# pinterest/rocksplicator

Hardware: AMD Instinct MI355X
Metric: replicated updates/sec (Put+Delete) at 1024 shards (higher is better)
Workload: dtype u8; 1 GPU; 1024shards_16Bkey_1024Bval_zipf0.99; key_len=16, val_len=1024, tick_updates=819200, parallelism=shard-parallel x1

## Files before the change

### rocksplicator_amd/csrc/engine.hip

```cpp
#include <hip/hip_runtime.h>

#define WB_UNALIGNED_OK 1

#include <algorithm>
#include <atomic>
#include <chrono>
#include <cstdio>
#include <cstring>
#include <deque>
#include <map>
#include <memory>
#include <mutex>
#include <string>
#include <thread>
#include <vector>

#include "../../include/rocksplicator_gpu.h"
#include "dev_buf.h"
#include "fold.h"
#include "host_store.h"
#include "part_copy.h"
#include "snappy.h"
#include "wb_format.h"

static thread_local std::string g_err;
extern "C" const char *gra_last_error(void) { return g_err.c_str(); }

#define HIP_TRY(x)                                                     \
  do {                                                                 \
    hipError_t _e = (x);                                               \
    if (_e != hipSuccess) {                                            \
      g_err = std::string(#x) + ": " + hipGetErrorString(_e);          \
      return GRA_ERR;                                                  \
    }                                                                  \
  } while (0)

namespace gra {

struct UpdDesc {
  uint64_t off;
  uint64_t base_seq;
  uint32_t len;
  uint32_t shard;
};
struct TickPlace {
  uint64_t cur;
  uint64_t hdr_off;
  uint64_t payload_off;
  uint64_t payload_bytes;
  uint32_t total_rec;
  uint32_t overflow;
};
struct SnapTask {
  uint64_t comp_off;
  uint64_t out_off;
  uint32_t comp_len;
  uint32_t ulen;
};
struct GroupDesc {
  uint32_t shard, first, n_upds, _pad;
};
struct DevRunDesc {
  uint64_t base_seq, last_seq;
  uint64_t cur;
  uint64_t hdr_off, payload_off;
  uint32_t n_entries, payload_bytes;
  uint32_t pay_rel_base;
  uint32_t shard;
};

__host__ __device__ inline uint2 add2(uint2 a, uint2 b) {
  return make_uint2(a.x + b.x, a.y + b.y);
}


constexpr uint32_t kSnapStage = 508;

__global__ void __launch_bounds__(256) k_snappy(
    const uint8_t *__restrict__ comp, const SnapTask *__restrict__ tasks,
    uint32_t n, uint8_t *__restrict__ scratch,
    uint32_t *__restrict__ err_ring, uint32_t tick) {
  __shared__ uint8_t lds[256 * (kSnapStage + 4)];
  uint32_t i = blockIdx.x * blockDim.x + threadIdx.x;
  if (i >= n) return;
  SnapTask t = tasks[i];
  uint8_t *dst = scratch + t.out_off;
  uint32_t r;
  if (t.comp_len <= kSnapStage) {
    uint8_t *mine = lds + threadIdx.x * (kSnapStage + 4);
    const uint8_t *src = comp + t.comp_off;
    for (uint32_t b = 0; b < t.comp_len; b += 16)
      *(uint4 *)(mine + b) = *(const uint4 *)(src + b);
    r = snp::decompress(mine, t.comp_len, dst, t.ulen);
  } else {
    r = snp::decompress(comp + t.comp_off, t.comp_len, dst, t.ulen);
  }
  if (r != t.ulen) {
    for (int b = 0; b < 13; b++) dst[b] = 0xFF;
    atomicAdd(&err_ring[tick % 64u], 1u);
  }
}

constexpr uint32_t kErrRing = 64;

constexpr uint32_t kRecCache = 2;

__device__ __forceinline__ uint2 block_scan256(uint2 v, uint2 *total) {
  __shared__ uint2 wsum[4];
  const uint32_t lane = threadIdx.x & 63u, w = threadIdx.x >> 6;
  uint2 inc = v;
  for (int ofs = 1; ofs < 64; ofs <<= 1) {
    uint32_t x = __shfl_up(inc.x, ofs, 64), y = __shfl_up(inc.y, ofs, 64);
    if (lane >= (uint32_t)ofs) inc = add2(inc, make_uint2(x, y));
  }
  if (lane == 63) wsum[w] = inc;
  __syncthreads();
  uint2 before = make_uint2(0, 0), tot = make_uint2(0, 0);
  for (uint32_t k = 0; k < 4; k++) {
    uint2 s = wsum[k];
    if (k < w) before = add2(before, s);
    tot = add2(tot, s);
  }
  *total = tot;
  return make_uint2(before.x + inc.x - v.x, before.y + inc.y - v.y);
}

constexpr uint32_t kDecodeWin = 48;
static_assert(kDecodeWin % 16 == 0, "window is staged in 16 B chunks");

__global__ void __launch_bounds__(256) k_decode(
    const uint8_t *__restrict__ blobs, const UpdDesc *__restrict__ descs,
    uint32_t n, wb::WalkTotals *__restrict__ totals, uint32_t max_rec,
    uint32_t *__restrict__ err_ring, uint32_t tick,
    uint2 *__restrict__ partial, uint2 *__restrict__ bsums,
    wb::Rec *__restrict__ reccache, uint8_t *__restrict__ ok_out) {
  __shared__ uint32_t stage[256 * (kDecodeWin + 4) / 4];
  uint32_t i = blockIdx.x * 256 + threadIdx.x;
  uint2 v = make_uint2(0, 0);
  if (i < n) {
    UpdDesc d = descs[i];
    const uint8_t *rep = blobs + d.off;
    uint32_t *row = stage + threadIdx.x * ((kDecodeWin + 4) / 4);
    const uint32_t nch = wb::win_chunks(d.len, kDecodeWin);
    uint4 c[kDecodeWin / 16];
#pragma unroll
    for (uint32_t k = 0; k < kDecodeWin / 16; k++)
      if (k < nch) c[k] = *(const uint4 *)(rep + 16 * k);
#pragma unroll
    for (uint32_t k = 0; k < kDecodeWin / 16; k++)
      if (k < nch) {
        row[4 * k + 0] = c[k].x;
        row[4 * k + 1] = c[k].y;
        row[4 * k + 2] = c[k].z;
        row[4 * k + 3] = c[k].w;
      }
    wb::WinSrc src = {(const uint8_t *)row, wb::win_bytes(d.len, kDecodeWin),
                      rep};
    wb::Rec *cache = reccache + (size_t)i * kRecCache;
    wb::WalkTotals t = wb::walk_src(src, d.len,
                                    [&](const wb::Rec &r, uint32_t idx) {
                                      if (idx < kRecCache) cache[idx] = r;
                                    });
    if (t.n_records > max_rec) t.ok = 0;
    totals[i] = t;
    ok_out[i] = (uint8_t)t.ok;
    if (!t.ok) atomicAdd(&err_ring[tick % kErrRing], 1u);
    if (t.ok) v = make_uint2(t.n_records, t.payload16);
  }
  uint2 tot;
  uint2 excl = block_scan256(v, &tot);
  if (i < n) partial[i] = excl;
  if (threadIdx.x == 255) bsums[blockIdx.x] = tot;
}

__global__ void k_scan2(uint2 *__restrict__ bsums, uint32_t nblocks,
                        uint64_t *__restrict__ cursor,
                        TickPlace *__restrict__ place, uint64_t cap, int ring,
                        uint32_t task_cap, uint32_t *__restrict__ err_ring,
                        uint32_t tick) {
  const uint32_t per = (nblocks + 255) / 256;
  const uint32_t lo = threadIdx.x * per < nblocks ? threadIdx.x * per : nblocks;
  const uint32_t hi = lo + per < nblocks ? lo + per : nblocks;
  uint2 mine = make_uint2(0, 0);
  for (uint32_t i = lo; i < hi; i++) mine = add2(mine, bsums[i]);
  uint2 carry;
  uint2 run = block_scan256(mine, &carry);
  for (uint32_t i = lo; i < hi; i++) {
    uint2 v = bsums[i];
    bsums[i] = run;
    run = add2(run, v);
  }
  if (threadIdx.x == 0) {
    bsums[nblocks] = carry;
    uint2 tot = carry;
    uint64_t need_hdr = (((uint64_t)tot.x * sizeof(wb::RecHdr)) + 15) & ~15ULL;
    uint64_t need_pay = tot.y;
    uint64_t need = need_hdr + need_pay;
    TickPlace p = {};
    p.total_rec = tot.x;
    p.payload_bytes = need_pay;
    uint64_t cur = *cursor;
    if ((cur % cap) + need > cap) cur += cap - (cur % cap);
    if (need > cap || (!ring && cur + need > cap) ||
        (uint64_t)tot.x * 2 > task_cap) {
      p.overflow = 1;
      p.total_rec = 0;
      atomicAdd(&err_ring[tick % kErrRing], 1u);
    } else {
      p.cur = cur;
      p.hdr_off = cur % cap;
      p.payload_off = (cur % cap) + need_hdr;
      *cursor = cur + need;
    }
    *place = p;
    err_ring[(tick + kErrRing / 2) % kErrRing] = 0;
  }
}

__global__ void k_emit(const uint8_t *__restrict__ blobs,
                       const UpdDesc *__restrict__ descs, uint32_t n,
                       const wb::WalkTotals *__restrict__ totals,
                       const uint2 *__restrict__ partial,
                       const uint2 *__restrict__ bsums,
                       const TickPlace *__restrict__ place,
                       uint8_t *__restrict__ store,
                       CopyTask *__restrict__ tasks,
                       const wb::Rec *__restrict__ reccache) {
  uint32_t i = blockIdx.x * blockDim.x + threadIdx.x;
  if (i >= n) return;
  if (place->overflow) return;
  wb::WalkTotals t = totals[i];
  if (!t.ok || t.n_records == 0) return;
  UpdDesc d = descs[i];
  uint2 base = add2(partial[i], bsums[i >> 8]);
  wb::RecHdr *hdrs = (wb::RecHdr *)(store + place->hdr_off);
  uint8_t *pay_region = store + place->payload_off;
  uint32_t pay = base.y;
  uint32_t rec = base.x;
  auto emit_one = [&](const wb::Rec &r, uint32_t idx) {
    uint32_t cf4 = r.cf_id ? 4u : 0u;
    uint8_t btag = wb::base_tag(r.tag);
    uint32_t cfv = (cf4 && btag == wb::kRangeDeletion) ? 4u : 0u;
    wb::RecHdr h;
    h.seq = d.base_seq + idx;
    h.kv_off = pay;
    h.val_len = r.val_len + cfv;
    h.key_len = (uint16_t)(r.key_len + cf4);
    h.type = btag;
    h.flags = cf4 ? 1 : 0;
    h.kpref = 0;
    hdrs[rec + idx] = h;
    if (cf4) {
      *(uint32_t *)(pay_region + pay) = r.cf_id;
    }
    CopyTask tk;
    tk.src_off = d.off + r.key_off;
    tk.dst_rel = pay + cf4;
    tk.nbytes = r.key_len;
    tasks[2 * (rec + idx)] = tk;
    if (cfv) {
      uint8_t *p = pay_region + pay + cf4 + r.key_len;
      p[0] = (uint8_t)r.cf_id;
      p[1] = (uint8_t)(r.cf_id >> 8);
      p[2] = (uint8_t)(r.cf_id >> 16);
      p[3] = (uint8_t)(r.cf_id >> 24);
    }
    tk.src_off = d.off + r.val_off;
    tk.dst_rel = pay + cf4 + r.key_len + cfv;
    tk.nbytes = r.val_len;
    tasks[2 * (rec + idx) + 1] = tk;
    pay += (cf4 + r.key_len + cfv + r.val_len + 15u) & ~15u;
  };
  if (t.n_records <= kRecCache) {
    const wb::Rec *cache = reccache + (size_t)i * kRecCache;
    for (uint32_t idx = 0; idx < t.n_records; idx++) emit_one(cache[idx], idx);
  } else {
    wb::walk_f(blobs + d.off, d.len, emit_one);
  }
}

template <int G>
__device__ __forceinline__ void copy_dword(uint8_t *dst, const uint8_t *src,
                                           uint32_t n, uint32_t lane) {
  uint32_t head = (uint32_t)((0u - (uint32_t)(uintptr_t)dst) & 3u);
  if (head > n) head = n;
  if (lane < head) dst[lane] = src[lane];
  dst += head;
  src += head;
  n -= head;
  uint32_t nw = n >> 2;
  uint32_t r = (uint32_t)((uintptr_t)src & 3);
  const uint32_t *asrc = (const uint32_t *)(src - r);
  uint32_t *adst = (uint32_t *)dst;
  if (r == 0) {
    for (uint32_t w = lane; w < nw; w += G) adst[w] = asrc[w];
  } else {
    uint32_t sh = 8 * r;
    for (uint32_t w = lane; w < nw; w += G)
      adst[w] = (asrc[w] >> sh) | (asrc[w + 1] << (32 - sh));
  }
  uint32_t done = nw << 2, tail = n & 3;
  if (lane < tail) dst[done + lane] = src[done + lane];
}

template <int G, int R, bool UNAL>
__global__ void __launch_bounds__(256) k_copy(const uint8_t *__restrict__ blobs,
                                              uint8_t *__restrict__ store,
                                              const TickPlace *__restrict__ place,
                                              const CopyTask *__restrict__ tasks) {
  if (place->overflow) return;
  uint32_t wave = (blockIdx.x * blockDim.x + threadIdx.x) >> 6;
  uint32_t nwaves = (gridDim.x * blockDim.x) >> 6;
  pcopy::part_copy<G, R, UNAL>(blobs, store + place->payload_off, tasks,
                               place->total_rec, wave, nwaves);
}

__global__ void k_drain(const uint8_t *__restrict__ store,
                        const TickPlace *__restrict__ place,
                        uint8_t *__restrict__ hostbuf) {
  if (place->overflow) return;
  uint64_t hdr_bytes = (uint64_t)place->total_rec * sizeof(wb::RecHdr);
  uint64_t hb16 = (hdr_bytes + 15) & ~15ull;
  uint64_t pay = place->payload_bytes;
  const uint8_t *hsrc = store + place->hdr_off;
  const uint8_t *psrc = store + place->payload_off;
  size_t stride = (size_t)gridDim.x * blockDim.x * 16;
  size_t i0 = ((size_t)blockIdx.x * blockDim.x + threadIdx.x) * 16;
  for (size_t b = i0; b < hdr_bytes; b += stride)
    *(uint4 *)(hostbuf + b) = *(const uint4 *)(hsrc + b);
  uint8_t *pdst = hostbuf + hb16;
  for (size_t b = i0; b < pay; b += stride)
    *(uint4 *)(pdst + b) = *(const uint4 *)(psrc + b);
}

__global__ void k_rundesc(const GroupDesc *__restrict__ groups, uint32_t ngroups,
                          const UpdDesc *__restrict__ descs,
                          const wb::WalkTotals *__restrict__ totals,
                          const uint2 *__restrict__ partial,
                          const uint2 *__restrict__ bsums, uint32_t n,
                          uint32_t nblocks,
                          const TickPlace *__restrict__ place,
                          DevRunDesc *__restrict__ out) {
  uint32_t g = blockIdx.x * blockDim.x + threadIdx.x;
  if (g >= ngroups) return;
  GroupDesc gd = groups[g];
  auto scan_at = [&](uint32_t j) {
    return j >= n ? bsums[nblocks] : add2(partial[j], bsums[j >> 8]);
  };
  uint2 s0 = scan_at(gd.first);
  uint2 s1 = scan_at(gd.first + gd.n_upds);
  DevRunDesc rd = {};
  rd.shard = gd.shard;
  rd.n_entries = s1.x - s0.x;
  rd.payload_bytes = s1.y - s0.y;
  rd.pay_rel_base = s0.y;
  if (!place->overflow) {
    rd.cur = place->cur;
    rd.hdr_off = place->hdr_off + (uint64_t)s0.x * sizeof(wb::RecHdr);
    rd.payload_off = place->payload_off + s0.y;
    rd.base_seq = descs[gd.first].base_seq;
    const UpdDesc last = descs[gd.first + gd.n_upds - 1];
    rd.last_seq = last.base_seq + totals[gd.first + gd.n_upds - 1].hdr_count - 1;
  } else {
    rd.n_entries = 0;
  }
  out[g] = rd;
}

#include "mg_kernels.h"

#include "scan_kernels.h"

#include "compact_kernels.h"

#include "reclaim_kernels.h"

__host__ __device__ inline uint64_t rec_hash_cs(uint64_t seq, uint8_t type,
                                                uint32_t klen, uint32_t vlen,
                                                const uint8_t *key,
                                                const uint8_t *val) {
  uint64_t h = 1469598103934665603ULL;
#define GRA_FOLD(b) h = (h ^ (uint8_t)(b)) * 1099511628211ULL
  for (int i = 0; i < 8; i++) GRA_FOLD(seq >> (8 * i));
  GRA_FOLD(type);
  for (int i = 0; i < 4; i++) GRA_FOLD(klen >> (8 * i));
  for (int i = 0; i < 4; i++) GRA_FOLD(vlen >> (8 * i));
  for (uint32_t i = 0; i < klen; i++) GRA_FOLD(key[i]);
  for (uint32_t i = 0; i < vlen; i++) GRA_FOLD(val[i]);
#undef GRA_FOLD
  return h;
}

__global__ void k_checksum(const uint8_t *__restrict__ store,
                           const RunView *__restrict__ runs, uint32_t nruns,
                           unsigned long long *__restrict__ out) {
  uint64_t local = 0;
  for (uint32_t r = blockIdx.x; r < nruns; r += gridDim.x) {
    RunView rv = runs[r];
    const wb::RecHdr *hdrs = (const wb::RecHdr *)(store + rv.hdr_off);
    const uint8_t *pay = store + rv.payload_off;
    for (uint32_t i = threadIdx.x; i < rv.n_entries; i += blockDim.x) {
      wb::RecHdr h = hdrs[i];
      uint32_t rel = h.kv_off - rv.pay_rel_base;
      local += rec_hash_cs(h.seq, h.type, h.key_len, h.val_len, pay + rel,
                           pay + rel + h.key_len);
    }
  }
  for (int ofs = 32; ofs > 0; ofs >>= 1)
    local += __shfl_down(local, ofs, 64);
  if ((threadIdx.x & 63) == 0 && local)
    atomicAdd(out, (unsigned long long)local);
}

static bool env_flag(const char *name) {
  const char *v = getenv(name);
  return v && v[0] == '1';
}

static bool gra_check_staging() {
  static const bool on = env_flag("GRA_CHECK_STAGING");
  return on;
}


struct Stats {
  double h2d_ms = 0, snappy_ms = 0, decode_ms = 0, scan_ms = 0, emit_ms = 0,
         copy_ms = 0, runfix_ms = 0, total_ms = 0;
  uint64_t ticks = 0, updates = 0, records = 0, blob_bytes = 0, payload_bytes = 0;
};

constexpr int kSlots = 8;
enum TickEvent {
  kEvTickStart,
  kEvH2dStart,
  kEvH2dDone,
  kEvSnappyStart,
  kEvSnappyDone,
  kEvAfterDecode,
  kEvAfterScan,
  kEvAfterEmit,
  kEvAfterCopy,
  kEvMainEnd,
  kEvPublished,
  kEventsPerTick
};

struct TickRec {
  int slot = -1;
  uint32_t n = 0, ngroups = 0;
  uint64_t blob_bytes = 0;
  uint32_t evmask = 0;
  std::vector<uint32_t> counts;
  std::shared_ptr<uint8_t> drain_buf;
  hipEvent_t ev[kEventsPerTick];

  hipError_t record(TickEvent k, hipStream_t s) {
    evmask |= bit(k);
    return hipEventRecord(ev[k], s);
  }
  bool has(TickEvent k) const { return evmask & bit(k); }
  static uint32_t bit(TickEvent k) { return 1u << k; }
};

struct TickInput {
  uint32_t n = 0;
  const std::vector<GroupDesc> *groups = nullptr;
  const GroupDesc *d_groups = nullptr;
  uint64_t blob_bytes = 0;
  std::vector<uint32_t> counts;
  const uint8_t *d_blobs = nullptr;
  const UpdDesc *d_descs = nullptr;
  const void *stage_src = nullptr;
  size_t stage_bytes = 0;
  const UpdDesc *h_descs = nullptr;
  const uint8_t *d_comp = nullptr;
  const SnapTask *d_snaptasks = nullptr;
  hipEvent_t window_ev = nullptr;
};

struct Slot {
  GroupDesc *h_groups = nullptr;
  TickPlace *h_place = nullptr;
  DevRunDesc *h_rundescs = nullptr;
  DevRunDesc *d_rundescs = nullptr;
  uint8_t *d_ok = nullptr;
  uint8_t *h_ok = nullptr;
  uint32_t *h_err = nullptr;
  UpdDesc *h_descs = nullptr;
  bool busy = false;
};

}

using namespace gra;

struct GraEngine {
  GraEngineOpts opts;
  hipStream_t stream = nullptr;
  hipStream_t copyout = nullptr;
  hipStream_t h2d = nullptr;
  hipStream_t prep = nullptr;
  uint8_t *d_store = nullptr;
  uint64_t *d_cursor = nullptr;
  uint32_t max_upd;
  uint32_t task_cap;
  uint32_t copy_grid;
  uint32_t group_cap;
  wb::WalkTotals *d_totals = nullptr;
  uint2 *d_partial = nullptr;
  uint2 *d_bsums = nullptr;
  wb::Rec *d_reccache = nullptr;
  CopyTask *d_tasks = nullptr;
  TickPlace *d_place = nullptr;
  GroupDesc *d_groups = nullptr;
  uint32_t *d_err_ring = nullptr;
  uint32_t tick_id = 0;
  static constexpr int kWriterSlots = 256;
  struct WriterSlot {
    alignas(64) std::atomic<uint32_t> n{0};
  };
  struct StageBuf {
    uint8_t *pin = nullptr;
    GraUpdateDesc *descs = nullptr;
    alignas(64) std::atomic<uint64_t> pos{0};
    alignas(64) std::atomic<uint32_t> nslots{0};
    alignas(64) std::atomic<bool> closed{false};
    alignas(64) std::atomic<uint32_t> staged{0};
    WriterSlot writers[kWriterSlots];
    uint64_t epoch = 0;
    hipEvent_t free_ev = nullptr;
  };
  StageBuf stage[2];
  std::atomic<StageBuf *> cur_stage{nullptr};
  uint8_t *d_stage_blobs_bufs[2] = {nullptr, nullptr};
  UpdDesc *d_stage_descs_bufs[2] = {nullptr, nullptr};
  hipEvent_t stage_used_ev[2] = {nullptr, nullptr};
  hipEvent_t h2d_gate_ev[2] = {nullptr, nullptr};
  Slot slots[kSlots];
  std::deque<TickRec> pending;
  std::vector<hipEvent_t> event_pool;
  struct MgCounts {
    uint32_t ncand, ntomb;
  };
  struct MgCache {
    DevBuf<RunView> d_runs;
    DevBuf<GraKeyRef> d_keys;
    DevBuf<uint8_t> d_keybuf, d_valbuf;
    DevBuf<GraGetResult> d_out;
    DevBuf<MgExtra> d_extra;
    DevBuf<uint64_t> d_qtab;
    DevBuf<MgCand> d_cands;
    DevBuf<MgTomb> d_tombs;
    DevBuf<unsigned long long> d_aux;
    DevMirror<MgCounts> counts;
  } mg;
  struct ScCache {
    DevBuf<RunView> d_runs;
    DevBuf<uint8_t> d_bounds, d_out;
    DevBuf<ScCand> d_cands;
    DevBuf<ScTomb> d_tombs;
    DevBuf<ScItem> d_items;
    DevBuf<ScHead> d_heads;
    DevBuf<ScFold> d_folds;
    DevBuf<ScSum> d_bsums;
    DevBuf<GraScanEntry> d_ents;
    DevMirror<ScCtl> ctl;
    DevMirror<CpCtl> cp;
    uint32_t cand_cap = 0;
  } sc;
  std::mutex drain_mu;
  std::vector<std::pair<uint8_t *, size_t>> drain_pool;
  bool closing = false;
  std::shared_ptr<uint8_t> drain_alloc(size_t need);
  std::vector<ShardState> shards;
  Stats stats;
  std::mutex mu;
  std::mutex maint_mu;
  std::atomic<uint64_t> store_epoch{0};
  uint64_t rc_bounce_bytes = 0, rc_piece_bytes = 0;
  DevBuf<uint8_t> rc_bounce;
  DevBuf<RcTask> rc_tasks;

  int init(const GraEngineOpts &o);
  ~GraEngine();
  int enqueue_tick(TickInput &in);
  int ingest(bool wait_all);
  int ingest_one(TickRec &t, bool wait);
  int flush_locked();
  int stream_tick_locked();
  hipEvent_t get_event();
  void put_event(hipEvent_t e);
  int free_slot();
};

struct GraDb {
  GraEngine *e;
  uint32_t shard;
};

struct TickPlan {
  std::vector<GroupDesc> groups;
  uint64_t blob_bytes = 0;
  GroupDesc *d_groups = nullptr;
  UpdDesc *d_ud = nullptr;
  hipEvent_t consumed_ev = nullptr;
  SnapTask *d_snap = nullptr;
};

struct GraReplay {
  GraEngine *e = nullptr;
  uint8_t *d_blobs = nullptr;
  bool external_blobs = false;
  UpdDesc *d_descs = nullptr;
  std::vector<UpdDesc> descs;
  std::vector<uint16_t> counts;
  size_t arena_bytes = 0;
  const uint8_t *h_arena = nullptr;
  uint8_t *d_comp = nullptr;
  SnapTask *d_snaptasks = nullptr;
  std::vector<SnapTask> snap_tasks;
  bool snappy = false;
  std::map<std::pair<uint64_t, uint64_t>, TickPlan> plans;
};

std::shared_ptr<uint8_t> GraEngine::drain_alloc(size_t need) {
  uint8_t *p = nullptr;
  size_t cap = 0;
  {
    std::lock_guard<std::mutex> lk(drain_mu);
    for (auto it = drain_pool.begin(); it != drain_pool.end(); ++it) {
      if (it->second >= need) {
        p = it->first;
        cap = it->second;
        drain_pool.erase(it);
        break;
      }
    }
  }
  if (!p) {
    cap = need + 64;
    if (hipHostMalloc(&p, cap) != hipSuccess) return nullptr;
  }
  GraEngine *e = this;
  return std::shared_ptr<uint8_t>(p, [e, cap](uint8_t *q) {
    std::lock_guard<std::mutex> lk(e->drain_mu);
    if (e->closing) {
      (void)hipHostFree(q);
    } else {
      e->drain_pool.push_back({q, cap});
    }
  });
}

hipEvent_t GraEngine::get_event() {
  if (!event_pool.empty()) {
    hipEvent_t e = event_pool.back();
    event_pool.pop_back();
    return e;
  }
  hipEvent_t e;
  (void)hipEventCreate(&e);
  return e;
}
void GraEngine::put_event(hipEvent_t e) { event_pool.push_back(e); }

int GraEngine::init(const GraEngineOpts &o) {
  opts = o;
  if (opts.store_bytes == 0) opts.store_bytes = 4ULL << 30;
  if (opts.staging_bytes == 0) opts.staging_bytes = 256ULL << 20;
  if (opts.max_wb_records == 0) opts.max_wb_records = 1024;
  max_upd = 1u << 20;
  task_cap = 4u << 20;
  copy_grid = 2048;
  if (const char *g = getenv("GRA_COPY_GRID")) {
    long v = atol(g);
    copy_grid = (uint32_t)(v < 1 ? 1 : v > 2048 ? 2048 : v);
  }
  rc_bounce_bytes = 64ull << 20;
  rc_piece_bytes = 16u << 20;
  if (const char *g = getenv("GRA_RECLAIM_BOUNCE"))
    rc_bounce_bytes = strtoull(g, nullptr, 10);
  if (const char *g = getenv("GRA_RECLAIM_PIECE"))
    rc_piece_bytes = strtoull(g, nullptr, 10);
  group_cap = opts.nshards + 1 > 65536 ? opts.nshards + 1 : 65536;
  (void)hipGetLastError();
  int ndev = 0;
  hipError_t de = hipGetDeviceCount(&ndev);
  if (de != hipSuccess || ndev == 0) {
    g_err = "no HIP device present — the GPU apply path refuses to run "
            "(no CPU fallback by design)";
    return GRA_NO_GPU;
  }
  if (opts.device >= 0) {
    hipError_t se = hipSetDevice(opts.device);
    if (se != hipSuccess) {
      g_err = std::string("hipSetDevice: ") + hipGetErrorString(se);
      (void)hipGetLastError();
      return GRA_ERR;
    }
  }
  HIP_TRY(hipStreamCreate(&stream));
  HIP_TRY(hipStreamCreate(&copyout));
  HIP_TRY(hipStreamCreate(&h2d));
  HIP_TRY(hipStreamCreate(&prep));
  HIP_TRY(hipMalloc(&d_store, opts.store_bytes + 16));
  HIP_TRY(hipMalloc(&d_cursor, 8));
  HIP_TRY(hipMemset(d_cursor, 0, 8));
  HIP_TRY(hipMalloc(&d_totals, (size_t)max_upd * sizeof(wb::WalkTotals)));
  HIP_TRY(hipMalloc(&d_partial, (size_t)max_upd * sizeof(uint2)));
  HIP_TRY(hipMalloc(&d_bsums, ((size_t)max_upd / 256 + 2) * sizeof(uint2)));
  HIP_TRY(hipMalloc(&d_reccache, (size_t)max_upd * 2 * sizeof(wb::Rec)));
  HIP_TRY(hipMalloc(&d_tasks, (size_t)task_cap * sizeof(CopyTask)));
  HIP_TRY(hipMalloc(&d_place, kSlots * sizeof(TickPlace)));
  HIP_TRY(hipMalloc(&d_groups, (size_t)group_cap * sizeof(GroupDesc)));
  HIP_TRY(hipMalloc(&d_err_ring, kErrRing * 4));
  HIP_TRY(hipMemset(d_err_ring, 0, kErrRing * 4));
  for (int i = 0; i < 2; i++) {
    HIP_TRY(hipMalloc(&d_stage_blobs_bufs[i], opts.staging_bytes + 16));
    HIP_TRY(hipMalloc(&d_stage_descs_bufs[i], (size_t)max_upd * sizeof(UpdDesc)));
    HIP_TRY(hipEventCreate(&stage_used_ev[i]));
    HIP_TRY(hipEventRecord(stage_used_ev[i], stream));
    HIP_TRY(hipEventCreateWithFlags(&h2d_gate_ev[i], hipEventDisableTiming));
    HIP_TRY(hipEventRecord(h2d_gate_ev[i], h2d));
  }
  static std::atomic<uint64_t> g_epoch{1};
  for (int i = 0; i < 2; i++) {
    HIP_TRY(hipHostMalloc(&stage[i].pin, opts.staging_bytes + 16,
                          hipHostMallocNonCoherent));
    stage[i].descs = (GraUpdateDesc *)malloc((size_t)max_upd * sizeof(GraUpdateDesc));
    stage[i].epoch = g_epoch.fetch_add(1u << 20);
    HIP_TRY(hipEventCreate(&stage[i].free_ev));
    HIP_TRY(hipEventRecord(stage[i].free_ev, stream));
  }
  cur_stage.store(&stage[0]);
  for (int i = 0; i < kSlots; i++) {
    Slot &s = slots[i];
    HIP_TRY(hipHostMalloc(&s.h_groups, (size_t)group_cap * sizeof(GroupDesc)));
    HIP_TRY(hipHostMalloc(&s.h_place, sizeof(TickPlace)));
    HIP_TRY(hipHostMalloc(&s.h_rundescs, (size_t)group_cap * sizeof(DevRunDesc)));
    HIP_TRY(hipMalloc(&s.d_rundescs, (size_t)group_cap * sizeof(DevRunDesc)));
    HIP_TRY(hipMalloc(&s.d_ok, (size_t)max_upd));
    HIP_TRY(hipHostMalloc(&s.h_ok, (size_t)max_upd));
    HIP_TRY(hipHostMalloc(&s.h_err, 4));
    HIP_TRY(hipHostMalloc(&s.h_descs, (size_t)max_upd * sizeof(UpdDesc)));
  }
  if (opts.drain_host && opts.store_ring &&
      opts.store_bytes < 10 * opts.staging_bytes) {
    g_err = "drain_host with store_ring needs store_bytes >= 10x "
            "staging_bytes (ring wrap inside the drain pipeline)";
    return GRA_ERR;
  }
  shards = std::vector<ShardState>(opts.nshards);
  event_pool.reserve(kSlots * kEventsPerTick);
  for (int i = 0; i < kSlots * kEventsPerTick; i++) {
    hipEvent_t ev;
    HIP_TRY(hipEventCreate(&ev));
    event_pool.push_back(ev);
  }
  return GRA_OK;
}

GraEngine::~GraEngine() {
  {
    std::lock_guard<std::mutex> lk(drain_mu);
    closing = true;
  }
  (void)hipStreamSynchronize(stream);
  (void)hipStreamSynchronize(copyout);
  (void)hipStreamSynchronize(h2d);
  for (auto &t : pending)
    for (int i = 0; i < kEventsPerTick; i++)
      if (t.ev[i]) (void)hipEventDestroy(t.ev[i]);
  for (auto e : event_pool) (void)hipEventDestroy(e);
  for (int i = 0; i < 2; i++) {
    if (stage[i].pin) (void)hipHostFree(stage[i].pin);
    free(stage[i].descs);
    if (stage[i].free_ev) (void)hipEventDestroy(stage[i].free_ev);
  }
  for (int i = 0; i < kSlots; i++) {
    Slot &s = slots[i];
    if (s.h_groups) (void)hipHostFree(s.h_groups);
    if (s.h_place) (void)hipHostFree(s.h_place);
    if (s.h_rundescs) (void)hipHostFree(s.h_rundescs);
    if (s.d_rundescs) (void)hipFree(s.d_rundescs);
    if (s.d_ok) (void)hipFree(s.d_ok);
    if (s.h_ok) (void)hipHostFree(s.h_ok);
    if (s.h_err) (void)hipHostFree(s.h_err);
    if (s.h_descs) (void)hipHostFree(s.h_descs);
  }
  for (int i = 0; i < 2; i++) {
    if (d_stage_blobs_bufs[i]) (void)hipFree(d_stage_blobs_bufs[i]);
    if (d_stage_descs_bufs[i]) (void)hipFree(d_stage_descs_bufs[i]);
    if (stage_used_ev[i]) (void)hipEventDestroy(stage_used_ev[i]);
    if (h2d_gate_ev[i]) (void)hipEventDestroy(h2d_gate_ev[i]);
  }
  for (void *p : {(void *)d_totals, (void *)d_partial, (void *)d_bsums,
                  (void *)d_reccache, (void *)d_store, (void *)d_cursor,
                  (void *)d_tasks,
                  (void *)d_place, (void *)d_groups, (void *)d_err_ring})
    if (p) (void)hipFree(p);
  shards.clear();
  pending.clear();
  {
    std::lock_guard<std::mutex> lk(drain_mu);
    for (auto &pr : drain_pool) (void)hipHostFree(pr.first);
    drain_pool.clear();
  }
  if (stream) (void)hipStreamDestroy(stream);
  if (copyout) (void)hipStreamDestroy(copyout);
  if (h2d) (void)hipStreamDestroy(h2d);
  if (prep) (void)hipStreamDestroy(prep);
}

int GraEngine::free_slot() {
  for (;;) {
    for (int i = 0; i < kSlots; i++)
      if (!slots[i].busy) return i;
    int rc = ingest(false);
    if (rc != GRA_OK) return -1;
    if (!pending.empty()) {
      if (ingest_one(pending.front(), true) != GRA_OK) return -1;
      pending.pop_front();
    }
  }
}

int GraEngine::enqueue_tick(TickInput &in) {
  const uint32_t n = in.n;
  const uint64_t blob_bytes = in.blob_bytes;
  const std::vector<GroupDesc> &groups = *in.groups;
  if (n == 0) return GRA_OK;
  if (n > max_upd) {
    g_err = "tick exceeds max updates per tick";
    return GRA_ERR;
  }
  if (opts.drain_host && opts.store_ring && blob_bytes * 10 > opts.store_bytes) {
    g_err = "drain_host with store_ring needs store_bytes >= 10x the tick "
            "size (ring wrap inside the drain pipeline)";
    return GRA_ERR;
  }
  if (groups.size() > group_cap) {
    g_err = "tick exceeds max shard-groups per tick";
    return GRA_ERR;
  }
  int si = free_slot();
  if (si < 0) return GRA_ERR;
  Slot &sl = slots[si];
  sl.busy = true;
  uint32_t ngroups = (uint32_t)groups.size();
  memcpy(sl.h_groups, groups.data(), ngroups * sizeof(GroupDesc));
  const GroupDesc *groups_for_kernel = in.d_groups ? in.d_groups : d_groups;
  uint32_t tick = tick_id++;

  TickRec t;
  t.slot = si;
  t.n = n;
  t.ngroups = ngroups;
  t.blob_bytes = blob_bytes;
  t.counts = std::move(in.counts);
  for (int i = 0; i < kEventsPerTick; i++) t.ev[i] = get_event();
  static const bool detailed = env_flag("GRA_DETAILED_EVENTS");

  if (!in.d_groups) {
    HIP_TRY(hipMemcpyAsync(d_groups, sl.h_groups, ngroups * sizeof(GroupDesc),
                           hipMemcpyHostToDevice, stream));
  }
  HIP_TRY(t.record(kEvTickStart, stream));
  const uint8_t *d_blobs = in.d_blobs;
  const UpdDesc *d_descw = in.d_descs;
  int stage_buf = -1;
  if (in.stage_src != nullptr) {
    stage_buf = (int)(tick & 1u);
    d_blobs = d_stage_blobs_bufs[stage_buf];
    if (in.h_descs) d_descw = d_stage_descs_bufs[stage_buf];
    HIP_TRY(hipEventSynchronize(h2d_gate_ev[stage_buf]));
    HIP_TRY(hipStreamWaitEvent(h2d, stage_used_ev[stage_buf], 0));
    HIP_TRY(t.record(kEvH2dStart, h2d));
    HIP_TRY(hipMemcpyAsync(d_stage_blobs_bufs[stage_buf], in.stage_src,
                           in.stage_bytes, hipMemcpyHostToDevice, h2d));
    if (in.h_descs) {
      memcpy(sl.h_descs, in.h_descs, (size_t)n * sizeof(UpdDesc));
      HIP_TRY(hipMemcpyAsync(d_stage_descs_bufs[stage_buf], sl.h_descs,
                             (size_t)n * sizeof(UpdDesc),
                             hipMemcpyHostToDevice, h2d));
    }
    HIP_TRY(t.record(kEvH2dDone, h2d));
    HIP_TRY(hipEventRecord(h2d_gate_ev[stage_buf], h2d));
    HIP_TRY(hipStreamWaitEvent(stream, t.ev[kEvH2dDone], 0));
  }
  uint32_t nb = (n + 255) / 256;
  if (in.d_snaptasks) {
    if (in.window_ev) HIP_TRY(hipStreamWaitEvent(prep, in.window_ev, 0));
    HIP_TRY(t.record(kEvSnappyStart, prep));
    hipLaunchKernelGGL(k_snappy, dim3(nb), dim3(256), 0, prep, in.d_comp,
                       in.d_snaptasks, n, (uint8_t *)d_blobs, d_err_ring,
                       tick);
    HIP_TRY(hipGetLastError());
    HIP_TRY(t.record(kEvSnappyDone, prep));
    HIP_TRY(hipStreamWaitEvent(stream, t.ev[kEvSnappyDone], 0));
  }
  hipLaunchKernelGGL(k_decode, dim3(nb), dim3(256), 0, stream, d_blobs,
                     d_descw, n, d_totals, opts.max_wb_records, d_err_ring,
                     tick, d_partial, d_bsums, d_reccache, sl.d_ok);
  HIP_TRY(hipGetLastError());
  if (detailed) HIP_TRY(t.record(kEvAfterDecode, stream));
  TickPlace *place_slot = d_place + si;
  hipLaunchKernelGGL(k_scan2, dim3(1), dim3(256), 0, stream, d_bsums, nb,
                     d_cursor, place_slot, opts.store_bytes, opts.store_ring,
                     task_cap, d_err_ring, tick);
  HIP_TRY(hipGetLastError());
  if (detailed) HIP_TRY(t.record(kEvAfterScan, stream));
  hipLaunchKernelGGL(k_emit, dim3(nb), dim3(256), 0, stream, d_blobs, d_descw,
                     n, d_totals, d_partial, d_bsums, place_slot, d_store,
                     d_tasks, d_reccache);
  HIP_TRY(hipGetLastError());
  HIP_TRY(t.record(kEvAfterEmit, stream));
  {
    const size_t avg = blob_bytes / n;
    const dim3 grid(copy_grid), blk(256);
    if (avg >= 768)
      hipLaunchKernelGGL((k_copy<64, 4, false>), grid, blk, 0, stream, d_blobs,
                         d_store, place_slot, d_tasks);
    else if (avg >= 384)
      hipLaunchKernelGGL((k_copy<32, 4, true>), grid, blk, 0, stream, d_blobs,
                         d_store, place_slot, d_tasks);
    else if (avg >= 192)
      hipLaunchKernelGGL((k_copy<16, 4, true>), grid, blk, 0, stream, d_blobs,
                         d_store, place_slot, d_tasks);
    else
      hipLaunchKernelGGL((k_copy<8, 4, true>), grid, blk, 0, stream, d_blobs,
                         d_store, place_slot, d_tasks);
  }
  HIP_TRY(hipGetLastError());
  HIP_TRY(t.record(kEvAfterCopy, stream));
  if (in.window_ev)
    HIP_TRY(hipEventRecord(in.window_ev, stream));
  hipLaunchKernelGGL(k_rundesc, dim3((ngroups + 255) / 256), dim3(256), 0,
                     stream, groups_for_kernel, ngroups, d_descw, d_totals,
                     d_partial, d_bsums, n, nb, place_slot, sl.d_rundescs);
  HIP_TRY(hipGetLastError());
  HIP_TRY(t.record(kEvMainEnd, stream));
  if (stage_buf >= 0)
    HIP_TRY(hipEventRecord(stage_used_ev[stage_buf], stream));
  HIP_TRY(hipStreamWaitEvent(copyout, t.ev[kEvMainEnd], 0));
  HIP_TRY(hipMemcpyAsync(sl.h_rundescs, sl.d_rundescs,
                         (size_t)ngroups * sizeof(DevRunDesc),
                         hipMemcpyDeviceToHost, copyout));
  HIP_TRY(hipMemcpyAsync(sl.h_err, d_err_ring + (tick % kErrRing), 4,
                         hipMemcpyDeviceToHost, copyout));
  HIP_TRY(hipMemcpyAsync(sl.h_place, place_slot, sizeof(TickPlace),
                         hipMemcpyDeviceToHost, copyout));
  if (opts.drain_host && !t.counts.empty()) {
    uint64_t recs = 0;
    for (uint32_t c : t.counts) recs += c;
    size_t need = (size_t)blob_bytes + 46 * recs + 80;
    t.drain_buf = drain_alloc(need);
    if (t.drain_buf) {
      hipLaunchKernelGGL(k_drain, dim3(1024), dim3(256), 0, copyout, d_store,
                         place_slot, t.drain_buf.get());
      HIP_TRY(hipGetLastError());
    }
  }
  HIP_TRY(t.record(kEvPublished, copyout));
  pending.push_back(std::move(t));
  return GRA_OK;
}

static int fetch_run_impl(GraEngine *e, Run &r);

static std::shared_ptr<Run> run_from(const DevRunDesc &rd, bool on_device) {
  auto run = std::make_shared<Run>();
  run->base_seq = rd.base_seq;
  run->last_seq = rd.last_seq;
  run->n_entries = rd.n_entries;
  run->payload_bytes = rd.payload_bytes;
  run->pay_rel_base = rd.pay_rel_base;
  if (on_device) {
    run->hdr_cur = rd.hdr_off;
    run->payload_cur = rd.payload_off;
  }
  return run;
}

static void roll_back_locked(ShardState &ss) {
  ss.next_seq = ss.durable_seq + 1;
  while (!ss.log.empty() && ss.log.back().base_seq > ss.durable_seq) {
    ss.log_used -= ss.log.back().rep.size();
    ss.log.pop_back();
  }
}

int GraEngine::ingest_one(TickRec &t, bool wait) {
  if (wait) {
    HIP_TRY(hipEventSynchronize(t.ev[kEvPublished]));
  } else {
    hipError_t q = hipEventQuery(t.ev[kEvPublished]);
    if (q == hipErrorNotReady) return GRA_NOT_FOUND;
    if (q != hipSuccess) {
      g_err = std::string("tick event: ") + hipGetErrorString(q);
      return GRA_ERR;
    }
  }
  Slot &sl = slots[t.slot];
  float ms;
  auto dt = [&](TickEvent a, TickEvent b) {
    if (!t.has(a) || !t.has(b)) return 0.0;
    (void)hipEventElapsedTime(&ms, t.ev[a], t.ev[b]);
    return (double)ms;
  };
  stats.h2d_ms += dt(kEvH2dStart, kEvH2dDone);
  stats.snappy_ms += dt(kEvSnappyStart, kEvSnappyDone);
  TickEvent prev = t.has(kEvH2dDone) ? kEvH2dDone : kEvTickStart;
  if (t.has(kEvAfterDecode)) {
    stats.decode_ms += dt(prev, kEvAfterDecode);
    prev = kEvAfterDecode;
  }
  if (t.has(kEvAfterScan)) {
    stats.scan_ms += dt(prev, kEvAfterScan);
    prev = kEvAfterScan;
  }
  stats.emit_ms += dt(prev, kEvAfterEmit);
  stats.copy_ms += dt(kEvAfterEmit, kEvAfterCopy);
  stats.runfix_ms += dt(kEvAfterCopy, kEvMainEnd);
  stats.total_ms += dt(kEvTickStart, kEvMainEnd);
  stats.ticks += 1;
  stats.updates += t.n;
  stats.blob_bytes += t.blob_bytes;
  uint32_t err = *sl.h_err;
  auto attach_drain = [&](Run &run, const DevRunDesc &rd) -> bool {
    if (!t.drain_buf || sl.h_place->overflow) return false;
    uint64_t hb16 =
        ((uint64_t)sl.h_place->total_rec * sizeof(wb::RecHdr) + 15) & ~15ull;
    run.hbuf = t.drain_buf;
    run.hdr_p = t.drain_buf.get() + (rd.hdr_off - sl.h_place->hdr_off);
    run.pay_p = t.drain_buf.get() + hb16;
    return true;
  };
  if (err != 0) {
    HIP_TRY(hipMemcpy(sl.h_ok, sl.d_ok, t.n, hipMemcpyDeviceToHost));
    const bool have_counts = t.counts.size() == t.n;
    for (uint32_t g = 0; g < t.ngroups; g++) {
      DevRunDesc &rd = sl.h_rundescs[g];
      const GroupDesc &gd = sl.h_groups[g];
      ShardState &ss = shards[rd.shard];
      std::lock_guard<std::mutex> lk(ss.mu);
      if (rd.base_seq == 0) {
        ss.poisoned = true;
        ss.cnt_failures++;
        roll_back_locked(ss);
        continue;
      }
      if (ss.poisoned) {
        roll_back_locked(ss);
        continue;
      }
      uint32_t keep_recs = 0;
      uint64_t keep_seq = rd.base_seq - 1;
      bool bad = false;
      for (uint32_t i = 0; i < gd.n_upds; i++) {
        if (!sl.h_ok[gd.first + i]) {
          bad = true;
          break;
        }
        uint32_t c = have_counts ? t.counts[gd.first + i] : 0;
        keep_recs += c;
        keep_seq += c;
      }
      if (!bad) {
        auto run = run_from(rd, true);
        if (opts.drain_host && !attach_drain(*run, rd))
          (void)fetch_run_impl(this, *run);
        if (rd.n_entries > 0 && !opts.store_ring) ss.runs.push_back(std::move(run));
        if (rd.last_seq > ss.durable_seq) ss.durable_seq = rd.last_seq;
        stats.records += rd.n_entries;
        stats.payload_bytes += rd.payload_bytes;
        continue;
      }
      if (keep_recs > 0 && have_counts && !opts.store_ring) {
        auto run = run_from(rd, true);
        run->last_seq = keep_seq;
        run->n_entries = keep_recs;
        if (opts.drain_host && !attach_drain(*run, rd))
          (void)fetch_run_impl(this, *run);
        ss.runs.push_back(std::move(run));
        stats.records += keep_recs;
      }
      if (keep_seq > ss.durable_seq) ss.durable_seq = keep_seq;
      ss.poisoned = true;
      ss.cnt_failures++;
      roll_back_locked(ss);
    }
  } else if (opts.store_ring) {
    for (uint32_t g = 0; g < t.ngroups; g++) {
// ... 1644 lines not shown
```

### rocksplicator_amd/csrc/wb_format.h

```cpp
#pragma once
#include <stdint.h>

#ifdef __HIP__
#define WB_HD __host__ __device__ inline
#define WB_HD_OP __host__ __device__
#else
#define WB_HD static inline
#define WB_HD_OP
#endif

namespace wb {

enum Tag : uint8_t {
  kDeletion = 0x00,
  kValue = 0x01,
  kMerge = 0x02,
  kLogData = 0x03,
  kCfDeletion = 0x04,
  kCfValue = 0x05,
  kCfMerge = 0x06,
  kSingleDeletion = 0x07,
  kCfSingleDeletion = 0x08,
  kBeginPrepare = 0x09,
  kEndPrepare = 0x0A,
// ... 63 lines not shown
                            uint32_t *out) {
  uint32_t result = 0;
#pragma unroll
  for (uint32_t i = 0; i < 5; i++) {
    if (i >= avail) return 0;
    uint32_t byte = src.byte(pos + i);
    if (byte & 0x80) {
      result |= (byte & 0x7F) << (7 * i);
    } else {
      if (i == 4 && byte > 0x0F) return 0;
      result |= byte << (7 * i);
      *out = result;
      return i + 1;
    }
  }
  return 0;
}
WB_HD uint32_t varint32(const uint8_t *p, uint32_t avail, uint32_t *out) {
  return varint32_src(PtrSrc{p}, 0, avail, out);
}

constexpr uint32_t kFnvBasis32 = 2166136261u;
WB_HD uint32_t key_fnv_fold(uint32_t h, const uint8_t *p, uint32_t n) {
  for (uint32_t i = 0; i < n; i++) h = (h ^ p[i]) * 16777619u;
  return h;
}

WB_HD bool consumes_seq(uint8_t tag) {
  switch (tag) {
    case kValue: case kDeletion: case kMerge: case kSingleDeletion:
    case kRangeDeletion: case kCfValue: case kCfDeletion: case kCfMerge:
    case kCfSingleDeletion: case kCfRangeDeletion:
      return true;
    default:
      return false;
  }
}
WB_HD bool has_cf_prefix(uint8_t tag) {
  return tag == kCfValue || tag == kCfDeletion || tag == kCfMerge ||
         tag == kCfSingleDeletion || tag == kCfRangeDeletion;
}
WB_HD uint8_t base_tag(uint8_t tag) {
  switch (tag) {
    case kCfValue: return kValue;
    case kCfDeletion: return kDeletion;
    case kCfMerge: return kMerge;
    case kCfSingleDeletion: return kSingleDeletion;
    case kCfRangeDeletion: return kRangeDeletion;
    default: return tag;
  }
}
WB_HD int nslices(uint8_t btag) {
  switch (btag) {
    case kValue: case kMerge: case kRangeDeletion: return 2;
    case kDeletion: case kSingleDeletion: return 1;
    case kLogData: return 2 - 1;
    case kEndPrepare: case kCommit: case kRollback: return 1;
    case kBeginPrepare: case kNoop: return 0;
    default: return -1;
  }
}

struct Rec {
  uint32_t key_off, key_len;
  uint32_t val_off, val_len;
  uint8_t tag;
  uint8_t consumes;
  uint16_t _pad;
  uint32_t cf_id;
};

struct WalkTotals {
  uint32_t n_records;
  uint32_t payload_bytes;
  uint32_t payload16;
  uint32_t hdr_count;
  uint32_t ok;
  uint32_t _pad;
  uint64_t hdr_seq;
};

template <class Src, class F>
WB_HD WalkTotals walk_src(const Src &src, uint32_t len, F &&f) {
  WalkTotals t = {0, 0, 0, 0, 0, 0, 0};
  if (len < kHeaderBytes) return t;
  t.hdr_seq = src.u64(0);
  t.hdr_count = src.u32(8);
  uint32_t pos = kHeaderBytes;
  uint32_t consumed = 0, nrec = 0, payload = 0, payload16 = 0;
  while (pos < len) {
    uint8_t tag = src.byte(pos++);
    uint8_t bt = base_tag(tag);
    int ns = nslices(bt);
    if (ns < 0) return t;
    uint32_t cf = 0;
    if (has_cf_prefix(tag)) {
      uint32_t c = varint32_src(src, pos, len - pos, &cf);
      if (c == 0) return t;
      pos += c;
    }
    uint32_t off[2] = {0, 0}, slen[2] = {0, 0};
    for (int s = 0; s < ns; s++) {
      uint32_t n, c = varint32_src(src, pos, len - pos, &n);
      if (c == 0) return t;
      pos += c;
      if (pos + n > len || n > len) return t;
      off[s] = pos;
      slen[s] = n;
      pos += n;
    }
    if (consumes_seq(tag)) {
      Rec r;
      r.key_off = off[0];
      r.key_len = slen[0];
      r.val_off = off[1];
      r.val_len = slen[1];
      r.tag = tag;
      r.consumes = 1;
      r._pad = 0;
      r.cf_id = cf;
      f(r, nrec);
      uint32_t cf4 = cf ? 4u : 0u;
      uint32_t cfx = (cf && bt == kRangeDeletion) ? 8u : cf4;
      payload += slen[0] + slen[1] + cfx;
      payload16 += (slen[0] + slen[1] + cfx + 15u) & ~15u;
      nrec++;
      consumed++;
    }
  }
  if (consumed != t.hdr_count) return t;
  t.n_records = nrec;
  t.payload_bytes = payload;
  t.payload16 = payload16;
  t.ok = 1;
  return t;
}

template <class F>
WB_HD WalkTotals walk_f(const uint8_t *rep, uint32_t len, F &&f) {
  return walk_src(PtrSrc{rep}, len, f);
}

struct NullEmit {
  WB_HD_OP void operator()(const Rec &, uint32_t) const {}
};

WB_HD WalkTotals walk(const uint8_t *rep, uint32_t len, Rec *emit, uint32_t cap) {
  if (!emit) return walk_f(rep, len, NullEmit{});
  return walk_f(rep, len, [&](const Rec &r, uint32_t i) {
    if (i < cap) emit[i] = r;
  });
}

struct RecHdr {
  uint64_t seq;
  uint32_t kv_off;
  uint32_t val_len;
  uint16_t key_len;
  uint8_t type;
  uint8_t flags;
  uint32_t kpref;
};

WB_HD uint32_t key_prefix4(const uint8_t *key, uint32_t klen) {
  uint32_t p = 0;
  for (uint32_t i = 0; i < 4 && i < klen; i++) p |= (uint32_t)key[i] << (8 * i);
  return p;
}
static_assert(sizeof(RecHdr) == 24, "RecHdr must be 24 bytes");

}
```

Before: 1.917 billion updates/s.

## Pack decode results into 16-byte EmitRec and fold run-desc into emit kernel

The decode kernel now writes one compact 16-byte EmitRec per update (single-record fast path or walk flag) instead of a 32-byte WalkTotals plus a two-entry Rec cache, which cuts global memory traffic between decode and emit. The separate k_rundesc launch is removed; its work runs in extra blocks appended to the k_emit grid, and it reads hdr_count directly from the blob header. Updates with two records now fall back to a re-walk of the blob, and val_gap packing assumes small gaps.

```diff
diff --git a/rocksplicator_amd/csrc/engine.hip b/rocksplicator_amd/csrc/engine.hip
--- a/rocksplicator_amd/csrc/engine.hip
+++ b/rocksplicator_amd/csrc/engine.hip
@@ -103,8 +103,6 @@
 
 constexpr uint32_t kErrRing = 64;
 
-constexpr uint32_t kRecCache = 2;
-
 __device__ __forceinline__ uint2 block_scan256(uint2 v, uint2 *total) {
   __shared__ uint2 wsum[4];
   const uint32_t lane = threadIdx.x & 63u, w = threadIdx.x >> 6;
@@ -130,10 +128,10 @@
 
 __global__ void __launch_bounds__(256) k_decode(
     const uint8_t *__restrict__ blobs, const UpdDesc *__restrict__ descs,
-    uint32_t n, wb::WalkTotals *__restrict__ totals, uint32_t max_rec,
+    uint32_t n, wb::EmitRec *__restrict__ emitrecs, uint32_t max_rec,
     uint32_t *__restrict__ err_ring, uint32_t tick,
     uint2 *__restrict__ partial, uint2 *__restrict__ bsums,
-    wb::Rec *__restrict__ reccache, uint8_t *__restrict__ ok_out) {
+    uint8_t *__restrict__ ok_out) {
   __shared__ uint32_t stage[256 * (kDecodeWin + 4) / 4];
   uint32_t i = blockIdx.x * 256 + threadIdx.x;
   uint2 v = make_uint2(0, 0);
@@ -156,13 +154,13 @@
       }
     wb::WinSrc src = {(const uint8_t *)row, wb::win_bytes(d.len, kDecodeWin),
                       rep};
-    wb::Rec *cache = reccache + (size_t)i * kRecCache;
+    wb::Rec first = {};
     wb::WalkTotals t = wb::walk_src(src, d.len,
                                     [&](const wb::Rec &r, uint32_t idx) {
-                                      if (idx < kRecCache) cache[idx] = r;
+                                      if (idx == 0) first = r;
                                     });
     if (t.n_records > max_rec) t.ok = 0;
-    totals[i] = t;
+    emitrecs[i] = wb::emit_pack(t, first);
     ok_out[i] = (uint8_t)t.ok;
     if (!t.ok) atomicAdd(&err_ring[tick % kErrRing], 1u);
     if (t.ok) v = make_uint2(t.n_records, t.payload16);
@@ -217,20 +215,59 @@
   }
 }
 
+__device__ __forceinline__ void run_desc(
+    uint32_t g, const uint8_t *__restrict__ blobs,
+    const GroupDesc *__restrict__ groups, const UpdDesc *__restrict__ descs,
+    const uint2 *__restrict__ partial, const uint2 *__restrict__ bsums,
+    uint32_t n, uint32_t nblocks, const TickPlace *__restrict__ place,
+    DevRunDesc *__restrict__ out) {
+  GroupDesc gd = groups[g];
+  auto scan_at = [&](uint32_t j) {
+    return j >= n ? bsums[nblocks] : add2(partial[j], bsums[j >> 8]);
+  };
+  uint2 s0 = scan_at(gd.first);
+  uint2 s1 = scan_at(gd.first + gd.n_upds);
+  DevRunDesc rd = {};
+  rd.shard = gd.shard;
+  rd.n_entries = s1.x - s0.x;
+  rd.payload_bytes = s1.y - s0.y;
+  rd.pay_rel_base = s0.y;
+  if (!place->overflow) {
+    rd.cur = place->cur;
+    rd.hdr_off = place->hdr_off + (uint64_t)s0.x * sizeof(wb::RecHdr);
+    rd.payload_off = place->payload_off + s0.y;
+    rd.base_seq = descs[gd.first].base_seq;
+    const UpdDesc last = descs[gd.first + gd.n_upds - 1];
+    const uint32_t hdr_count =
+        last.len >= wb::kHeaderBytes ? wb::fixed32_le(blobs + last.off + 8) : 0u;
+    rd.last_seq = last.base_seq + hdr_count - 1;
+  } else {
+    rd.n_entries = 0;
+  }
+  out[g] = rd;
+}
+
 __global__ void k_emit(const uint8_t *__restrict__ blobs,
                        const UpdDesc *__restrict__ descs, uint32_t n,
-                       const wb::WalkTotals *__restrict__ totals,
+                       const wb::EmitRec *__restrict__ emitrecs,
                        const uint2 *__restrict__ partial,
                        const uint2 *__restrict__ bsums,
                        const TickPlace *__restrict__ place,
                        uint8_t *__restrict__ store,
-                       CopyTask *__restrict__ tasks,
-                       const wb::Rec *__restrict__ reccache) {
+                       CopyTask *__restrict__ tasks, uint32_t nb,
+                       const GroupDesc *__restrict__ groups, uint32_t ngroups,
+                       DevRunDesc *__restrict__ rundescs) {
+  if (blockIdx.x >= nb) {
+    uint32_t g = (blockIdx.x - nb) * blockDim.x + threadIdx.x;
+    if (g < ngroups)
+      run_desc(g, blobs, groups, descs, partial, bsums, n, nb, place, rundescs);
+    return;
+  }
   uint32_t i = blockIdx.x * blockDim.x + threadIdx.x;
   if (i >= n) return;
   if (place->overflow) return;
-  wb::WalkTotals t = totals[i];
-  if (!t.ok || t.n_records == 0) return;
+  wb::EmitRec er = emitrecs[i];
+  if (er.kind == wb::kEmitNone) return;
   UpdDesc d = descs[i];
   uint2 base = add2(partial[i], bsums[i >> 8]);
   wb::RecHdr *hdrs = (wb::RecHdr *)(store + place->hdr_off);
@@ -271,9 +308,8 @@
     tasks[2 * (rec + idx) + 1] = tk;
     pay += (cf4 + r.key_len + cfv + r.val_len + 15u) & ~15u;
   };
-  if (t.n_records <= kRecCache) {
-    const wb::Rec *cache = reccache + (size_t)i * kRecCache;
-    for (uint32_t idx = 0; idx < t.n_records; idx++) emit_one(cache[idx], idx);
+  if (er.kind == wb::kEmitOne) {
+    emit_one(wb::emit_unpack(er), 0);
   } else {
     wb::walk_f(blobs + d.off, d.len, emit_one);
   }
@@ -333,40 +369,6 @@
     *(uint4 *)(pdst + b) = *(const uint4 *)(psrc + b);
 }
 
-__global__ void k_rundesc(const GroupDesc *__restrict__ groups, uint32_t ngroups,
-                          const UpdDesc *__restrict__ descs,
-                          const wb::WalkTotals *__restrict__ totals,
-                          const uint2 *__restrict__ partial,
-                          const uint2 *__restrict__ bsums, uint32_t n,
-                          uint32_t nblocks,
-                          const TickPlace *__restrict__ place,
-                          DevRunDesc *__restrict__ out) {
-  uint32_t g = blockIdx.x * blockDim.x + threadIdx.x;
-  if (g >= ngroups) return;
-  GroupDesc gd = groups[g];
-  auto scan_at = [&](uint32_t j) {
-    return j >= n ? bsums[nblocks] : add2(partial[j], bsums[j >> 8]);
-  };
-  uint2 s0 = scan_at(gd.first);
-  uint2 s1 = scan_at(gd.first + gd.n_upds);
-  DevRunDesc rd = {};
-  rd.shard = gd.shard;
-  rd.n_entries = s1.x - s0.x;
-  rd.payload_bytes = s1.y - s0.y;
-  rd.pay_rel_base = s0.y;
-  if (!place->overflow) {
-    rd.cur = place->cur;
-    rd.hdr_off = place->hdr_off + (uint64_t)s0.x * sizeof(wb::RecHdr);
-    rd.payload_off = place->payload_off + s0.y;
-    rd.base_seq = descs[gd.first].base_seq;
-    const UpdDesc last = descs[gd.first + gd.n_upds - 1];
-    rd.last_seq = last.base_seq + totals[gd.first + gd.n_upds - 1].hdr_count - 1;
-  } else {
-    rd.n_entries = 0;
-  }
-  out[g] = rd;
-}
-
 #include "mg_kernels.h"
 
 #include "scan_kernels.h"
@@ -506,10 +508,9 @@
   uint32_t task_cap;
   uint32_t copy_grid;
   uint32_t group_cap;
-  wb::WalkTotals *d_totals = nullptr;
+  wb::EmitRec *d_emitrecs = nullptr;
   uint2 *d_partial = nullptr;
   uint2 *d_bsums = nullptr;
-  wb::Rec *d_reccache = nullptr;
   CopyTask *d_tasks = nullptr;
   TickPlace *d_place = nullptr;
   GroupDesc *d_groups = nullptr;
@@ -706,10 +707,9 @@
   HIP_TRY(hipMalloc(&d_store, opts.store_bytes + 16));
   HIP_TRY(hipMalloc(&d_cursor, 8));
   HIP_TRY(hipMemset(d_cursor, 0, 8));
-  HIP_TRY(hipMalloc(&d_totals, (size_t)max_upd * sizeof(wb::WalkTotals)));
+  HIP_TRY(hipMalloc(&d_emitrecs, (size_t)max_upd * sizeof(wb::EmitRec)));
   HIP_TRY(hipMalloc(&d_partial, (size_t)max_upd * sizeof(uint2)));
   HIP_TRY(hipMalloc(&d_bsums, ((size_t)max_upd / 256 + 2) * sizeof(uint2)));
-  HIP_TRY(hipMalloc(&d_reccache, (size_t)max_upd * 2 * sizeof(wb::Rec)));
   HIP_TRY(hipMalloc(&d_tasks, (size_t)task_cap * sizeof(CopyTask)));
   HIP_TRY(hipMalloc(&d_place, kSlots * sizeof(TickPlace)));
   HIP_TRY(hipMalloc(&d_groups, (size_t)group_cap * sizeof(GroupDesc)));
@@ -794,9 +794,8 @@
     if (stage_used_ev[i]) (void)hipEventDestroy(stage_used_ev[i]);
     if (h2d_gate_ev[i]) (void)hipEventDestroy(h2d_gate_ev[i]);
   }
-  for (void *p : {(void *)d_totals, (void *)d_partial, (void *)d_bsums,
-                  (void *)d_reccache, (void *)d_store, (void *)d_cursor,
-                  (void *)d_tasks,
+  for (void *p : {(void *)d_emitrecs, (void *)d_partial, (void *)d_bsums,
+                  (void *)d_store, (void *)d_cursor, (void *)d_tasks,
                   (void *)d_place, (void *)d_groups, (void *)d_err_ring})
     if (p) (void)hipFree(p);
   shards.clear();
@@ -900,8 +899,8 @@
     HIP_TRY(hipStreamWaitEvent(stream, t.ev[kEvSnappyDone], 0));
   }
   hipLaunchKernelGGL(k_decode, dim3(nb), dim3(256), 0, stream, d_blobs,
-                     d_descw, n, d_totals, opts.max_wb_records, d_err_ring,
-                     tick, d_partial, d_bsums, d_reccache, sl.d_ok);
+                     d_descw, n, d_emitrecs, opts.max_wb_records, d_err_ring,
+                     tick, d_partial, d_bsums, sl.d_ok);
   HIP_TRY(hipGetLastError());
   if (detailed) HIP_TRY(t.record(kEvAfterDecode, stream));
   TickPlace *place_slot = d_place + si;
@@ -910,9 +909,10 @@
                      task_cap, d_err_ring, tick);
   HIP_TRY(hipGetLastError());
   if (detailed) HIP_TRY(t.record(kEvAfterScan, stream));
-  hipLaunchKernelGGL(k_emit, dim3(nb), dim3(256), 0, stream, d_blobs, d_descw,
-                     n, d_totals, d_partial, d_bsums, place_slot, d_store,
-                     d_tasks, d_reccache);
+  hipLaunchKernelGGL(k_emit, dim3(nb + (ngroups + 255) / 256), dim3(256), 0,
+                     stream, d_blobs, d_descw, n, d_emitrecs, d_partial,
+                     d_bsums, place_slot, d_store, d_tasks, nb,
+                     groups_for_kernel, ngroups, sl.d_rundescs);
   HIP_TRY(hipGetLastError());
   HIP_TRY(t.record(kEvAfterEmit, stream));
   {
@@ -935,10 +935,6 @@
   HIP_TRY(t.record(kEvAfterCopy, stream));
   if (in.window_ev)
     HIP_TRY(hipEventRecord(in.window_ev, stream));
-  hipLaunchKernelGGL(k_rundesc, dim3((ngroups + 255) / 256), dim3(256), 0,
-                     stream, groups_for_kernel, ngroups, d_descw, d_totals,
-                     d_partial, d_bsums, n, nb, place_slot, sl.d_rundescs);
-  HIP_TRY(hipGetLastError());
   HIP_TRY(t.record(kEvMainEnd, stream));
   if (stage_buf >= 0)
     HIP_TRY(hipEventRecord(stage_used_ev[stage_buf], stream));
diff --git a/rocksplicator_amd/csrc/wb_format.h b/rocksplicator_amd/csrc/wb_format.h
--- a/rocksplicator_amd/csrc/wb_format.h
+++ b/rocksplicator_amd/csrc/wb_format.h
@@ -239,6 +239,60 @@
   });
 }
 
+enum EmitKind : uint8_t {
+  kEmitNone = 0,
+  kEmitOne = 1,
+  kEmitWalk = 2,
+};
+
+constexpr uint8_t kEmitNoValue = 0;
+
+struct alignas(16) EmitRec {
+  uint32_t val_len;
+  uint32_t cf_id;
+  uint16_t key_len;
+  uint8_t key_off;
+  uint8_t val_gap;
+  uint8_t tag;
+  uint8_t kind;
+  uint16_t _pad;
+};
+static_assert(sizeof(EmitRec) == 16, "EmitRec must be 16 bytes");
+
+WB_HD EmitRec emit_pack(const WalkTotals &t, const Rec &first) {
+  EmitRec e = {0, 0, 0, 0, 0, 0, kEmitNone, 0};
+  if (!t.ok || t.n_records == 0) return e;
+  if (t.n_records != 1 || first.key_off > 255u || first.key_len > 65535u) {
+    e.kind = kEmitWalk;
+    return e;
+  }
+  e.val_len = first.val_len;
+  e.cf_id = first.cf_id;
+  e.key_len = (uint16_t)first.key_len;
+  e.key_off = (uint8_t)first.key_off;
+  e.val_gap = first.val_off
+                  ? (uint8_t)(first.val_off - (first.key_off + first.key_len))
+                  : kEmitNoValue;
+  e.tag = first.tag;
+  e.kind = kEmitOne;
+  return e;
+}
+
+WB_HD Rec emit_unpack(const EmitRec &e) {
+  Rec r;
+  r.key_off = e.key_off;
+  r.key_len = e.key_len;
+  r.val_off = e.val_gap != kEmitNoValue
+                  ? (uint32_t)e.key_off + e.key_len + e.val_gap
+                  : 0u;
+  r.val_len = e.val_len;
+  r.tag = e.tag;
+  r.consumes = 1;
+  r._pad = 0;
+  r.cf_id = e.cf_id;
+  return r;
+}
+
 struct RecHdr {
   uint64_t seq;
   uint32_t kv_off;
```

Measured after the change: 2.011 billion updates/s (median of 6 runs). 4.9% higher.
